# antgroup/ant-ray

Measured on NVIDIA H100. Metric: resnet50_ddp_train_images_per_sec, higher is better.
Workload: dtype bf16

## Files before the change

### ant-ray_b200/csrc/inst_norm.cu

```cuda
#include <algorithm>
#include <initializer_list>
#include <type_traits>

#include "norm_act.cuh"
#include "norm_cat.cuh"
#include "norm_infer.cuh"
#include "norm_kernels.cuh"
#include "norm_launch.h"
#include "norm_pool2.cuh"
#include "norm_res.cuh"
#include "norm_shuffle.cuh"
#include "norm_slice.cuh"

namespace b200c {
namespace bn {

static int ceil_div(int a, int b) { return (a + b - 1) / b; }

static int last_pow2(unsigned n) {
  n |= (n >> 1);
  n |= (n >> 2);
  n |= (n >> 4);
  n |= (n >> 8);
  n |= (n >> 16);
  return std::max<int>(1, n - (n >> 1));
}

static void reduce_config(int reduction, int stride, dim3* block, dim3* grid) {
  int block_x = std::min(last_pow2(stride), kTileW);
  int block_y = std::min(last_pow2(ceil_div(reduction, kElemsPerThread)), kMaxBlock / block_x);
  if (block_x * block_y != kMaxBlock) block_x = std::min(last_pow2(stride), kMaxBlock / block_y);
  int grid_y = std::min(ceil_div(reduction, block_y * kElemsPerThread), kMaxHBlock);
  *block = dim3(block_x, block_y, 1);
  *grid = dim3(ceil_div(stride, block_x), grid_y < 8 ? 1 : grid_y, 1);
}

static_assert(kEwVec % kStatsVec == 0, "vec_ok covers the statistics kernel's vector width");
static bool vec_ok(int stride, const void* const* ptrs, int n) {
  if (stride % kEwVec) return false;
  for (int i = 0; i < n; i++)
    if (reinterpret_cast<uintptr_t>(ptrs[i]) % 16) return false;
  return true;
}

constexpr size_t kBlockSmem = 48 * 1024;
constexpr size_t kStatsStaticSmem = 3 * kMaxBlock * 4 + 16;
constexpr size_t kBwdStaticSmem = 2 * kMaxBlock * 4 + 16;

static size_t stats_ring_bytes(dim3 block) {
  return (size_t)kStatsStages * kParallelLoads * block.x * block.y * sizeof(BVec<kStatsVec>);
}
static_assert(kStatsStaticSmem + (size_t)kStatsStages * kParallelLoads * (kMaxBlock / kStatsVec) * sizeof(BVec<kStatsVec>) <= kBlockSmem,
              "the statistics ring fits every block");

static_assert(kBwdStaticSmem + (size_t)kBwdStagesWide * 5 * kParallelLoads * (kMaxBlock / kBwdVec) * sizeof(BVec<kBwdVec>) <= kBlockSmem &&
                  kBwdStaticSmem + (size_t)kBwdStages * 2 * kParallelLoads * (kMaxBlock / kBwdVec) * sizeof(BVec<kBwdVec>) <= kBlockSmem,
              "the backward ring fits every block: 2 stages of up to 5 operands, 3 of 2");
struct BwdReduceLaunch {
  dim3 block, grid;
  int vec;
  size_t smem;
};
static BwdReduceLaunch bwd_reduce_launch(int m, int c, GradSrc src, bool dy2, bool dual, const void* const* ptrs, int n) {
  BwdReduceLaunch l;
  reduce_config(m, c, &l.block, &l.grid);
  l.vec = 1;
  l.smem = 0;
  if (src == kGradPool || !vec_ok(c, ptrs, n)) return l;
  const int ops = bwd_ring_operands(src == kGradY, dy2, dual);
  const size_t ring = (size_t)bwd_ring_stages(ops) * ops * kParallelLoads * (l.block.x / kBwdVec) * l.block.y * sizeof(BVec<kBwdVec>);
  l.block.x /= kBwdVec;
  l.vec = kBwdVec;
  l.smem = ring;
  return l;
}

static void ew_config(int reduction, int stride, int vec, dim3* block, dim3* grid) {
  const int groups = stride / vec;
  const int bx = std::min(groups, kEwThreads);
  const int by = kEwThreads / bx;
  const int gx = ceil_div(groups, bx);
  const int gy = std::max(1, std::min(ceil_div(reduction, by), 4096 / gx));
  *block = dim3(bx, by, 1);
  *grid = dim3(gx, gy, 1);
}

constexpr int kSemaphores = kMaxChannels / kTileW;
constexpr size_t kSemaphoreBytes = (size_t)kSemaphores * 4;

size_t scratch_bytes(int stride) {
  return kSemaphoreBytes + (size_t)3 * stride * kMaxHBlock * 4 + (size_t)2 * stride * 4;
}

struct Scratch {
  int* semaphores;
  float* staging;
  float* sums;
};
static Scratch carve(void* scratch, int stride) {
  char* p = static_cast<char*>(scratch);
  Scratch s;
  s.semaphores = reinterpret_cast<int*>(p);
  s.staging = reinterpret_cast<float*>(p + kSemaphoreBytes);
  s.sums = s.staging + (size_t)3 * stride * kMaxHBlock;
  return s;
}

template <int... Cs, typename F>
static auto with_const(int key, F&& f) {
  std::common_type_t<decltype(f(std::integral_constant<int, Cs>{}))...> kernel = nullptr;
  ((key == Cs ? void(kernel = f(std::integral_constant<int, Cs>{})) : void()), ...);
  return kernel;
}

using StatsKernel = void (*)(const bf16*, StatsOut, volatile float*, int*, int, int);
using SyncStatsKernel = void (*)(const bf16*, float*, float, volatile float*, int*, int, int);
using StatsDualKernel = void (*)(const bf16*, const bf16*, StatsOut, StatsOut, volatile float*, volatile float*, int*, int, int);
using TransformKernel = void (*)(const bf16*, const bf16*, bf16*, uint8_t*, const float*, const float*, const float*, const float*,
                                 const float*, const float*, const float*, const float*, int, int);
using PoolFwdKernel = void (*)(const bf16*, bf16*, uint8_t*, const float*, const float*, const float*, const float*, PoolDims, int, int);
using BwdReduceKernel = void (*)(const bf16*, const bf16*, const bf16*, const bf16*, const uint8_t*, bf16*, const float*, const float*,
                                 float*, float*, float*, float*, volatile float*, int*, PoolDims, const bf16*, const float*, const float*,
                                 float*, float*, float*, int, int, int);
using BwdElemtKernel = void (*)(const bf16*, const bf16*, const bf16*, const uint8_t*, const bf16*, bf16*, const float*, const float*,
                                const float*, const float*, const float*, const float*, float, const bf16*, bf16*, const float*,
                                const float*, const float*, const float*, int, int);

static StatsKernel stats_kernel(int vec) {
  return with_const<1, kStatsVec>(vec, [](auto v) -> StatsKernel { return k_bn_stats<decltype(v)::value>; });
}
static StatsDualKernel stats_dual_kernel(int vec) {
  return with_const<1, kStatsVec>(vec, [](auto v) -> StatsDualKernel { return k_bn_stats_dual<decltype(v)::value>; });
}
static SyncStatsKernel sync_stats_kernel(int vec) {
  return with_const<1, kStatsVec>(vec, [](auto v) -> SyncStatsKernel { return k_bn_sync_stats<decltype(v)::value>; });
}
static TransformKernel transform_kernel(int vec, int tail) {
  return with_const<1, kEwVec>(vec, [&](auto v) {
    return with_const<kTailNone, kTailRelu, kTailAddRelu, kTailBnAddRelu>(
        tail, [](auto t) -> TransformKernel { return k_bn_transform<decltype(v)::value, (Tail) decltype(t)::value>; });
  });
}
static PoolFwdKernel pool_fwd_kernel(int vec) {
  return with_const<1, kEwVec>(vec, [](auto v) -> PoolFwdKernel { return k_bn_pool_fwd<decltype(v)::value>; });
}
static BwdReduceKernel bwd_reduce_kernel(int src, bool dual) {
  if (dual)
    return with_const<kGradY, kGradBits>(src, [](auto g) -> BwdReduceKernel { return k_bn_bwd_reduce<(GradSrc) decltype(g)::value, true>; });
  return with_const<kGradY, kGradBits, kGradDy, kGradPool>(
      src, [](auto g) -> BwdReduceKernel { return k_bn_bwd_reduce<(GradSrc) decltype(g)::value, false>; });
}
static BwdElemtKernel bwd_elemt_kernel(int vec, int src, bool fct_ptr, bool dual) {
  return with_const<1, kEwVec>(vec, [&](auto v) {
    if (dual)
// ... 159 lines not shown
      if (vec == 1) load(act_bwd_reduce_kernel(act));
      load(act_transform_kernel(vec, act));
      load(act_infer_kernel<float>(vec, act));
      load(act_infer_kernel<bf16>(vec, act));
    }
    for (bool b : {false, true}) {
      load(res_transform_kernel(vec, b));
      load(res_infer_kernel<float>(vec, b));
      load(res_infer_kernel<bf16>(vec, b));
    }
  }
  return e;
}

constexpr cudaError_t kNoKernel = cudaErrorInvalidDeviceFunction;

static cudaError_t launch_stats(const FwdArgs& a, float* sync_row, cudaStream_t st) {
  Scratch s = carve(a.scratch, a.c);
  dim3 block, grid;
  reduce_config(a.m, a.c, &block, &grid);
  const int vec = vec_ok(a.c, &a.x, 1) ? kStatsVec : 1;
  block.x /= vec;
  const size_t smem = vec == kStatsVec ? stats_ring_bytes(block) : 0;
  const bf16* x = static_cast<const bf16*>(a.x);
  if (sync_row) {
    const SyncStatsKernel k = sync_stats_kernel(vec);
    if (!k) return kNoKernel;
    k<<<grid, block, smem, st>>>(x, sync_row, a.eps, s.staging, s.semaphores, a.m, a.c);
  } else {
    const StatsKernel k = stats_kernel(vec);
    if (!k) return kNoKernel;
    StatsOut o{a.save_mean, a.save_invstd, a.running_mean, a.running_var, a.num_batches_tracked, a.momentum,
               (float)((double)a.m / (double)(a.m - 1)), a.eps};
    k<<<grid, block, smem, st>>>(x, o, s.staging, s.semaphores, a.m, a.c);
  }
  return cudaGetLastError();
}

static cudaError_t launch_transform(const FwdArgs& a, cudaStream_t st) {
  const void* ptrs[3] = {a.x, a.y, a.identity ? a.identity : a.x};
  const int vec = vec_ok(a.c, ptrs, 3) ? kEwVec : 1;
  dim3 block, grid;
  ew_config(a.m, a.c, vec, &block, &grid);
  const TransformKernel k = transform_kernel(vec, !a.relu ? kTailNone : a.identity ? kTailAddRelu : kTailRelu);
  if (!k) return kNoKernel;
  k<<<grid, block, 0, st>>>(static_cast<const bf16*>(a.x), static_cast<const bf16*>(a.identity), static_cast<bf16*>(a.y),
                            static_cast<uint8_t*>(a.mask), a.save_mean, a.save_invstd, a.weight, a.bias, nullptr, nullptr, nullptr,
                            nullptr, a.m, a.c);
  return cudaGetLastError();
}

static PoolDims pool_dims(int h, int w) { return PoolDims{h, w, (h - 1) / 2 + 1, (w - 1) / 2 + 1}; }

static cudaError_t launch_pool_fwd(const FwdArgs& a, cudaStream_t st) {
  const PoolDims d = pool_dims(a.pool_h, a.pool_w);
  const int pooled_rows = a.m / (a.pool_h * a.pool_w) * d.oh * d.ow;
  const void* ptrs[3] = {a.x, a.y, a.argmax};
  const int vec = vec_ok(a.c, ptrs, 3) ? kEwVec : 1;
  dim3 block, grid;
  ew_config(pooled_rows, a.c, vec, &block, &grid);
  const PoolFwdKernel k = pool_fwd_kernel(vec);
  if (!k) return kNoKernel;
  k<<<grid, block, 0, st>>>(static_cast<const bf16*>(a.x), static_cast<bf16*>(a.y), static_cast<uint8_t*>(a.argmax), a.save_mean,
                            a.save_invstd, a.weight, a.bias, d, pooled_rows, a.c);
  return cudaGetLastError();
}

cudaError_t forward(const FwdArgs& a, cudaStream_t st) {
  const cudaError_t e = launch_stats(a, nullptr, st);
  if (e != cudaSuccess) return e;
  return a.pool_h ? launch_pool_fwd(a, st) : launch_transform(a, st);
}

static GradSrc grad_src(const BwdArgs& a, bool reduced) {
  if (!a.relu) return kGradDy;
  if (reduced && a.dy_masked) return kGradMasked;
  if (a.pool_h) return kGradPool;
  return a.mask ? kGradBits : kGradY;
}

static cudaError_t launch_bwd_reduce(const BwdArgs& a, cudaStream_t st) {
  Scratch s = carve(a.scratch, a.c);
  const GradSrc src = grad_src(a, false);
  const void* ptrs[5] = {a.x, a.dy, a.dy2 ? a.dy2 : a.dy, src == kGradY ? a.y : a.dy, a.dy_masked ? a.dy_masked : a.dy};
  const BwdReduceLaunch l = bwd_reduce_launch(a.m, a.c, src, a.dy2 != nullptr, false, ptrs, 5);
  const BwdReduceKernel k = bwd_reduce_kernel(src, false);
  if (!k) return kNoKernel;
  const void* mask = src == kGradPool ? a.argmax : a.mask;
  k<<<l.grid, l.block, l.smem, st>>>(static_cast<const bf16*>(a.x), static_cast<const bf16*>(a.dy), static_cast<const bf16*>(a.dy2),
                            static_cast<const bf16*>(a.y), static_cast<const uint8_t*>(mask), static_cast<bf16*>(a.dy_masked),
                            a.save_mean, a.save_invstd, s.sums, s.sums + a.c, a.grad_weight, a.grad_bias, s.staging, s.semaphores,
                            pool_dims(a.pool_h, a.pool_w), nullptr, nullptr, nullptr, nullptr, nullptr, nullptr, a.m, a.c, l.vec);
  return cudaGetLastError();
}

static cudaError_t launch_bwd_elemt(const BwdArgs& a, cudaStream_t st) {
  Scratch s = carve(a.scratch, a.c);
  const GradSrc src = grad_src(a, true);
  const void* g = src == kGradMasked ? a.dy_masked : a.dy;
  const void* ptrs[5] = {a.x, a.dx, g, a.dy2 && src != kGradMasked ? a.dy2 : a.dy, a.y};
  const int vec = vec_ok(a.c, ptrs, src == kGradY ? 5 : 4) ? kEwVec : 1;
  dim3 block, grid;
  ew_config(a.m, a.c, vec, &block, &grid);
  const BwdElemtKernel k = bwd_elemt_kernel(vec, src, a.norm_fct != nullptr, false);
  if (!k) return kNoKernel;
  k<<<grid, block, 0, st>>>(static_cast<const bf16*>(g), static_cast<const bf16*>(a.dy2), static_cast<const bf16*>(a.y),
                            static_cast<const uint8_t*>(a.mask), static_cast<const bf16*>(a.x), static_cast<bf16*>(a.dx), a.save_mean,
                            a.save_invstd, a.weight, s.sums, s.sums + a.c, a.norm_fct, (float)(1.0 / a.m), nullptr, nullptr, nullptr,
                            nullptr, nullptr, nullptr, a.m, a.c);
  return cudaGetLastError();
}

cudaError_t backward(const BwdArgs& a, cudaStream_t st) {
  const cudaError_t e = launch_bwd_reduce(a, st);
  return e == cudaSuccess ? launch_bwd_elemt(a, st) : e;
}

static size_t dual_extra_offset(int c) { return (scratch_bytes(c) + 15) / 16 * 16; }
size_t dual_scratch_bytes(int c) { return dual_extra_offset(c) + (size_t)3 * c * kMaxHBlock * 4 + (size_t)c * 4; }
static float* dual_staging(void* scratch, int c) { return reinterpret_cast<float*>(static_cast<char*>(scratch) + dual_extra_offset(c)); }
static float* dual_sum_xmu2(void* scratch, int c) { return dual_staging(scratch, c) + (size_t)3 * c * kMaxHBlock; }

static cudaError_t launch_stats_dual(const FwdArgs& a, const FwdArgs& b, cudaStream_t st) {
  Scratch s = carve(a.scratch, a.c);
  dim3 block, grid;
  reduce_config(a.m, a.c, &block, &grid);
  const void* xs[2] = {a.x, b.x};
  const int svec = vec_ok(a.c, xs, 2) ? kStatsVec : 1;
  block.x /= svec;
  grid.z = 2;
  const size_t smem = svec == kStatsVec ? stats_ring_bytes(block) : 0;
  const StatsDualKernel ks = stats_dual_kernel(svec);
  if (!ks) return kNoKernel;
  StatsOut oa{a.save_mean, a.save_invstd, a.running_mean, a.running_var, a.num_batches_tracked, a.momentum,
              (float)((double)a.m / (double)(a.m - 1)), a.eps};
  StatsOut ob{b.save_mean, b.save_invstd, b.running_mean, b.running_var, b.num_batches_tracked, b.momentum,
              (float)((double)b.m / (double)(b.m - 1)), b.eps};
  ks<<<grid, block, smem, st>>>(static_cast<const bf16*>(a.x), static_cast<const bf16*>(b.x), oa, ob, s.staging,
                             dual_staging(a.scratch, a.c), s.semaphores, a.m, a.c);
  return cudaGetLastError();
}

cudaError_t forward_dual(const FwdArgs& a, const FwdArgs& b, cudaStream_t st) {
  const cudaError_t e = launch_stats_dual(a, b, st);
  if (e != cudaSuccess) return e;
  dim3 block, grid;
  const void* ptrs[3] = {a.x, a.y, b.x};
  const int vec = vec_ok(a.c, ptrs, 3) ? kEwVec : 1;
  ew_config(a.m, a.c, vec, &block, &grid);
  const TransformKernel kt = transform_kernel(vec, kTailBnAddRelu);
  if (!kt) return kNoKernel;
  kt<<<grid, block, 0, st>>>(static_cast<const bf16*>(a.x), static_cast<const bf16*>(b.x), static_cast<bf16*>(a.y),
                             static_cast<uint8_t*>(a.mask), a.save_mean, a.save_invstd, a.weight, a.bias, b.save_mean, b.save_invstd,
                             b.weight, b.bias, a.m, a.c);
  return cudaGetLastError();
}

cudaError_t backward_dual(const BwdArgs& a, const BwdArgs& b, cudaStream_t st) {
  Scratch s = carve(a.scratch, a.c);
  float* sum2 = dual_sum_xmu2(a.scratch, a.c);
  const GradSrc src = a.mask ? kGradBits : kGradY;
  const void* rptrs[5] = {a.x, a.dy, a.dy2 ? a.dy2 : a.dy, src == kGradY ? a.y : a.dy, b.x};
  const BwdReduceLaunch l = bwd_reduce_launch(a.m, a.c, src, a.dy2 != nullptr, true, rptrs, 5);
  const BwdReduceKernel kr = bwd_reduce_kernel(src, true);
  if (!kr) return kNoKernel;
  kr<<<l.grid, l.block, l.smem, st>>>(static_cast<const bf16*>(a.x), static_cast<const bf16*>(a.dy), static_cast<const bf16*>(a.dy2),
                             static_cast<const bf16*>(a.y), static_cast<const uint8_t*>(a.mask), nullptr, a.save_mean, a.save_invstd,
                             s.sums, s.sums + a.c, a.grad_weight, a.grad_bias, s.staging, s.semaphores, pool_dims(0, 0),
// ... 439 lines not shown
```

### ant-ray_b200/csrc/norm_kernels.cuh

```cuda
#pragma once
#include <cuda_bf16.h>
#include <cuda_runtime.h>
#include <stdint.h>

#include <type_traits>

namespace b200c {
namespace bn {

constexpr int kMaxBlock = 512;
constexpr int kParallelLoads = 4;
constexpr int kElemsPerThread = 16;
constexpr int kTileW = 32;
constexpr int kMaxHBlock = 128;
constexpr int kStatsVec = 4;
constexpr int kBwdVec = 4;
constexpr int kStatsStages = 4;
constexpr unsigned kBwdStages = 3;
constexpr unsigned kBwdStagesWide = 2;
__host__ __device__ constexpr unsigned bwd_ring_stages(int ops) { return ops >= 3 ? kBwdStagesWide : kBwdStages; }
__host__ __device__ constexpr int bwd_ring_operands(bool y, bool dy2, bool dual) { return 2 + dy2 + y + dual; }
constexpr int kEwThreads = 256;
constexpr int kEwVec = 8;

typedef __nv_bfloat16 bf16;

template <int V>
struct alignas(2 * V) BVec {
  bf16 v[V];
};

__device__ __forceinline__ unsigned char* ring_smem() {
  extern __shared__ __align__(16) unsigned char bn_ring[];
  return bn_ring;
}
template <int BYTES>
__device__ __forceinline__ void cp_async(void* smem, const void* gmem) {
  asm volatile("cp.async.ca.shared.global [%0], [%1], %2;\n" ::"r"((unsigned)__cvta_generic_to_shared(smem)), "l"(gmem), "n"(BYTES)
               : "memory");
}
__device__ __forceinline__ void cp_async_commit() { asm volatile("cp.async.commit_group;\n" ::: "memory"); }
template <int N>
__device__ __forceinline__ void cp_async_wait() { asm volatile("cp.async.wait_group %0;\n" ::"n"(N) : "memory"); }


template <bool FUSE_NEW>
__device__ __forceinline__ void welford_merge_element(int& count, float& mean, float& m2n, const int& count_new,
                                                      const float& mean_new, const float& m2n_new) {
  float factor = float(1.0) / ::max(1, (count + count_new));
  float delta0 = mean - mean_new;
  const float c = count, c_new = count_new;
  mean = __fmul_rn(FUSE_NEW ? __fmaf_rn(mean_new, c_new, __fmul_rn(mean, c)) : __fmaf_rn(mean, c, __fmul_rn(mean_new, c_new)),
                   factor);
  m2n = __fadd_rn(m2n, __fmaf_rn(__fmul_rn(__fmul_rn(__fmul_rn(delta0, delta0), c_new), c), factor, m2n_new));
  count += count_new;
}

template <int V>
__device__ __forceinline__ void welford_merge_block_vertical(int (&count)[V], float (&mean)[V], float (&m2n)[V],
                                                             int* shmem_count, float* shmem_mean, float* shmem_m2n) {
  const int block_x = blockDim.x * V;
  auto address_base = threadIdx.x * V + threadIdx.y * block_x;
#pragma unroll
  for (int offset = blockDim.y / 2; offset > 0; offset >>= 1) {
    if (threadIdx.y < offset * 2) {
#pragma unroll
      for (int k = 0; k < V; k++) {
        shmem_mean[address_base + k] = mean[k];
        shmem_m2n[address_base + k] = m2n[k];
        shmem_count[address_base + k] = count[k];
      }
    }
    __syncthreads();
    if (threadIdx.y < offset && threadIdx.y + offset < blockDim.y) {
      auto address = address_base + offset * block_x;
#pragma unroll
      for (int k = 0; k < V; k++) {
        auto count_new = shmem_count[address + k];
        auto mean_new = shmem_mean[address + k];
        auto m2n_new = shmem_m2n[address + k];
        welford_merge_element<false>(count[k], mean[k], m2n[k], count_new, mean_new, m2n_new);
      }
    }
  }
}

template <int V>
__device__ __forceinline__ void merge_block_vertical_backward(float (&sum_dy)[V], float (&sum_dy_xmu)[V], float* shmem_sum_dy,
                                                              float* shmem_sum_dy_xmu) {
  const int block_x = blockDim.x * V;
  auto address_base = threadIdx.x * V + threadIdx.y * block_x;
#pragma unroll
  for (int offset = blockDim.y / 2; offset > 0; offset >>= 1) {
    if (threadIdx.y < offset * 2) {
#pragma unroll
      for (int k = 0; k < V; k++) {
        shmem_sum_dy[address_base + k] = sum_dy[k];
        shmem_sum_dy_xmu[address_base + k] = sum_dy_xmu[k];
      }
    }
    __syncthreads();
    if (threadIdx.y < offset && threadIdx.y + offset < blockDim.y) {
      auto address = address_base + offset * block_x;
// ... 304 lines not shown
#pragma unroll
    for (int j = 0; j < V; j++) {
      auto tmp = w_c[j] * (__bfloat162float(xv.v[j]) - m_c[j]) * inv_std_c[j] + s_c[j];
      if (TAIL == kTailAddRelu || BN2) {
        if (BN2) zv.v[j] = __float2bfloat16(w2_c[j] * (__bfloat162float(zv.v[j]) - m2_c[j]) * inv_std2_c[j] + s2_c[j]);
        const bf16 r = __float2bfloat16(__bfloat162float(__float2bfloat16(tmp)) + __bfloat162float(zv.v[j]));
        yv.v[j] = __bfloat162float(r) <= 0.f ? __float2bfloat16(0.f) : r;
      } else if (TAIL == kTailRelu) {
        yv.v[j] = tmp <= 0.f ? __float2bfloat16(0.f) : __float2bfloat16(tmp);
      } else {
        yv.v[j] = __float2bfloat16(tmp);
      }
      bits |= (unsigned)!(__bfloat162float(yv.v[j]) <= 0.f) << j;
    }
    *reinterpret_cast<BVec<V>*>(out + a) = yv;
    if (TAIL != kTailNone && mask) {
      if (V == 1) bits = (__ballot_sync(group, bits) >> (lane & ~7u)) & 0xffu;
      if (V == 8 || lane % 8 == 0) mask[a >> 3] = (uint8_t)bits;
    }
  }
}

struct PoolDims {
  int h, w, oh, ow;
};
constexpr uint8_t kPoolNoGrad = 0xff;

template <int V>
__global__ void __launch_bounds__(kEwThreads) k_bn_pool_fwd(const bf16* __restrict__ input, bf16* __restrict__ out,
                                                            uint8_t* __restrict__ argmax, const float* __restrict__ mean,
                                                            const float* __restrict__ inv_std, const float* __restrict__ weight,
                                                            const float* __restrict__ shift, const PoolDims d, const int pooled_rows,
                                                            const int stride) {
  const int c0 = (blockIdx.x * blockDim.x + threadIdx.x) * V;
  if (c0 >= stride) return;
  float m_c[V], inv_std_c[V], w_c[V], s_c[V];
#pragma unroll
  for (int j = 0; j < V; j++) {
    m_c[j] = mean[c0 + j];
    inv_std_c[j] = inv_std[c0 + j];
    w_c[j] = weight[c0 + j];
    s_c[j] = shift[c0 + j];
  }
  const int row_step = blockDim.y * gridDim.y;
  for (int p = blockIdx.y * blockDim.y + threadIdx.y; p < pooled_rows; p += row_step) {
    const int pw = p % d.ow, ph = (p / d.ow) % d.oh, n = p / (d.ow * d.oh);
    float best[V];
    uint8_t pos[V];
#pragma unroll
    for (int j = 0; j < V; j++) {
      best[j] = -INFINITY;
      pos[j] = 0;
    }
    for (int ih = max(2 * ph - 1, 0); ih < min(2 * ph + 2, d.h); ih++) {
      for (int iw = max(2 * pw - 1, 0); iw < min(2 * pw + 2, d.w); iw++) {
        const BVec<V> xv = *reinterpret_cast<const BVec<V>*>(input + ((size_t)(n * d.h + ih) * d.w + iw) * stride + c0);
        const uint8_t at = (ih - 2 * ph + 1) * 3 + (iw - 2 * pw + 1);
#pragma unroll
        for (int j = 0; j < V; j++) {
          const auto tmp = w_c[j] * (__bfloat162float(xv.v[j]) - m_c[j]) * inv_std_c[j] + s_c[j];
          const float y = __bfloat162float(tmp <= 0.f ? __float2bfloat16(0.f) : __float2bfloat16(tmp));
          if (y > best[j] || isnan(y)) {
            best[j] = y;
            pos[j] = at;
          }
        }
      }
    }
    BVec<V> yv;
    struct alignas(V) {
      uint8_t v[V];
    } av;
#pragma unroll
    for (int j = 0; j < V; j++) {
      yv.v[j] = __float2bfloat16(best[j]);
      av.v[j] = best[j] <= 0.f ? kPoolNoGrad : pos[j];
    }
    const size_t a = (size_t)p * stride + c0;
    *reinterpret_cast<BVec<V>*>(out + a) = yv;
    *reinterpret_cast<decltype(av)*>(argmax + a) = av;
  }
}

__device__ __forceinline__ bf16 pool_grad(const bf16* __restrict__ dpool, const uint8_t* __restrict__ argmax, const PoolDims& d,
                                          const int m, const int c, const int stride) {
  const int iw = m % d.w, ih = (m / d.w) % d.h, n = m / (d.w * d.h);
  const int ph0 = ih >> 1, ph1 = min((ih + 1) >> 1, d.oh - 1);
  const int pw0 = iw >> 1, pw1 = min((iw + 1) >> 1, d.ow - 1);
  const int o = ((n * d.oh + ph0) * d.ow + pw0) * stride + c;
  const int dr = (ph1 - ph0) * d.ow * stride, dc = (pw1 - pw0) * stride;
  const uint8_t a[4] = {argmax[o], argmax[o + dc], argmax[o + dr], argmax[o + dr + dc]};
  const bf16 v[4] = {dpool[o], dpool[o + dc], dpool[o + dr], dpool[o + dr + dc]};
  const int at = (ih - 2 * ph0 + 1) * 3 + (iw - 2 * pw0 + 1);
  if (ph0 == ph1 && pw0 == pw1) return a[0] == at ? v[0] : __float2bfloat16(0.f);
  float sum = 0.f;
  if (a[0] == at) sum += __bfloat162float(v[0]);
  if (pw1 != pw0 && a[1] == at - 2) sum += __bfloat162float(v[1]);
  if (ph1 != ph0 && a[2] == at - 6) sum += __bfloat162float(v[2]);
  if (ph1 != ph0 && pw1 != pw0 && a[3] == at - 8) sum += __bfloat162float(v[3]);
  return __float2bfloat16(sum);
}

__device__ __forceinline__ bf16 relu_grad(bf16 dy, bf16 y) { return __bfloat162float(y) <= 0.f ? __float2bfloat16(0.f) : dy; }
__device__ __forceinline__ bf16 relu_grad_bit(bf16 dy, unsigned bit) { return bit ? dy : __float2bfloat16(0.f); }
__device__ __forceinline__ bf16 add_grads(bf16 a, bf16 b) { return __float2bfloat16(__bfloat162float(a) + __bfloat162float(b)); }

enum GradSrc { kGradMasked, kGradY, kGradBits, kGradDy, kGradPool };
constexpr int kGradSrcs = 5;

template <GradSrc G, bool DUAL>
__global__ void __launch_bounds__(kMaxBlock) k_bn_bwd_reduce(const bf16* __restrict__ input, const bf16* __restrict__ grad_output,
                                const bf16* __restrict__ grad_output2, const bf16* __restrict__ output,
                                const uint8_t* __restrict__ mask, bf16* __restrict__ masked, const float* __restrict__ mean,
                                const float* __restrict__ inv_std, float* __restrict__ sum_dy_o, float* __restrict__ sum_dy_xmu_o,
                                float* __restrict__ grad_weight, float* __restrict__ grad_bias, volatile float* staging_data,
                                int* semaphores, const PoolDims pool, const bf16* __restrict__ input2,
                                const float* __restrict__ mean2, const float* __restrict__ inv_std2, float* __restrict__ sum_dy_xmu2_o,
                                float* __restrict__ grad_weight2, float* __restrict__ grad_bias2, const int reduction_size,
                                const int stride, const int vec) {
  static_assert(G != kGradMasked, "the reduce kernel computes g");
  constexpr bool BITS = G == kGradBits;
  constexpr bool POOL = G == kGradPool;
  constexpr int PARALLEL_LOADS = kParallelLoads;
  __shared__ float shmem_sum_dy[kMaxBlock];
  __shared__ float shmem_sum_dy_xmu[kMaxBlock];
  __shared__ bool is_last_block_done;

  auto body = [&](auto vec_c) {
    constexpr int V = decltype(vec_c)::value;
    float sum_dy[PARALLEL_LOADS][V];
    float sum_dy_xmu[PARALLEL_LOADS][V];
    float sum_dy_xmu2[PARALLEL_LOADS][V];
#pragma unroll
    for (int i = 0; i < PARALLEL_LOADS; i++) {
#pragma unroll
      for (int k = 0; k < V; k++) {
        sum_dy[i][k] = float(0);
        sum_dy_xmu[i][k] = float(0);
        sum_dy_xmu2[i][k] = float(0);
      }
    }
    int inner_loop_stride = blockDim.y * gridDim.y;
    int m_offset = blockIdx.y * blockDim.y + threadIdx.y;
    int c_offset = (blockIdx.x * blockDim.x + threadIdx.x) * V;
    if (c_offset >= stride || m_offset >= reduction_size) return;

    int loop_count = 1 + (reduction_size - 1) / (inner_loop_stride * PARALLEL_LOADS);
    int address_base = m_offset * stride + c_offset;
    int address_increment = inner_loop_stride * stride;
    float r_mean[V], factor[V], r_mean2[V];
#pragma unroll
    for (int k = 0; k < V; k++) {
      r_mean[k] = mean[c_offset + k];
      factor[k] = inv_std[c_offset + k];
      r_mean2[k] = DUAL ? mean2[c_offset + k] : 0.f;
    }

    auto consume = [&](int j, const BVec<V>* dy_p, const BVec<V>* dy2_p, const BVec<V>* y_p, uint8_t mask_byte, const BVec<V>* x_p,
                       const BVec<V>* x2_p) {
      float x_input[V], x_input2[V], x_grad_output[V];
      if (m_offset < reduction_size) {
        const unsigned bits = BITS ? mask_byte >> (address_base & 7) : 0u;
        BVec<V> gv;
#pragma unroll
        for (int k = 0; k < V; k++) {
          const bf16 dy = !POOL && grad_output2 ? add_grads(dy_p->v[k], dy2_p->v[k]) : dy_p->v[k];
          gv.v[k] = BITS ? relu_grad_bit(dy, (bits >> k) & 1u) : G == kGradY ? relu_grad(dy, y_p->v[k]) : dy;
          x_input[k] = __bfloat162float(x_p->v[k]);
          x_input2[k] = DUAL ? __bfloat162float(x2_p->v[k]) : 0.f;
          x_grad_output[k] = __bfloat162float(gv.v[k]);
        }
        if (masked) *reinterpret_cast<BVec<V>*>(masked + address_base) = gv;
      } else {
#pragma unroll
        for (int k = 0; k < V; k++) {
          x_input[k] = float(0);
          x_input2[k] = float(0);
          x_grad_output[k] = float(0);
        }
      }
      m_offset += inner_loop_stride;
      address_base += address_increment;
#pragma unroll
      for (int k = 0; k < V; k++) {
        sum_dy[j][k] += x_grad_output[k];
        sum_dy_xmu[j][k] = __fmaf_rn(x_grad_output[k], x_input[k] - r_mean[k], sum_dy_xmu[j][k]);
        if (DUAL) sum_dy_xmu2[j][k] = __fmaf_rn(x_grad_output[k], x_input2[k] - r_mean2[k], sum_dy_xmu2[j][k]);
      }
    };

    if constexpr (V == 1) {
      for (int i = 0; i < loop_count; i++) {
        BVec<V> dy_v[PARALLEL_LOADS], dy2_v[PARALLEL_LOADS], y_v[PARALLEL_LOADS], x_v[PARALLEL_LOADS], x2_v[PARALLEL_LOADS];
        uint8_t mask_v[PARALLEL_LOADS];
#pragma unroll
        for (int j = 0; j < PARALLEL_LOADS; j++) {
          if (m_offset + j * inner_loop_stride < reduction_size) {
            const int a = address_base + j * address_increment;
            if (POOL) dy_v[j].v[0] = pool_grad(grad_output, mask, pool, m_offset + j * inner_loop_stride, c_offset, stride);
            else dy_v[j].v[0] = grad_output[a];
            if (grad_output2) dy2_v[j].v[0] = grad_output2[a];
            if (BITS) mask_v[j] = mask[a >> 3];
            else if (G == kGradY) y_v[j].v[0] = output[a];
            x_v[j].v[0] = input[a];
            if (DUAL) x2_v[j].v[0] = input2[a];
          }
        }
#pragma unroll
        for (int j = 0; j < PARALLEL_LOADS; j++) consume(j, &dy_v[j], &dy2_v[j], &y_v[j], mask_v[j], &x_v[j], &x2_v[j]);
      }
    } else {
      const int ops = bwd_ring_operands(G == kGradY, grad_output2 != nullptr, DUAL);
      auto ring_walk = [&](auto stages_c) {
        constexpr unsigned D = decltype(stages_c)::value;
        const int threads = blockDim.x * blockDim.y;
        const int op_dy2 = 2, op_y = op_dy2 + (grad_output2 != nullptr), op_x2 = op_y + (G == kGradY);
        BVec<V>* ring = reinterpret_cast<BVec<V>*>(ring_smem()) + threadIdx.y * blockDim.x + threadIdx.x;
        auto stage = [&](unsigned it) { return ring + (it % D) * ops * PARALLEL_LOADS * threads; };
        const int first_row = m_offset;
        const int iteration_rows = PARALLEL_LOADS * inner_loop_stride;
        auto issue = [&](unsigned it) {
          BVec<V>* slot = stage(it);
          int m = first_row + (int)it * iteration_rows;
#pragma unroll
          for (int j = 0; j < PARALLEL_LOADS; j++, m += inner_loop_stride, slot += threads) {
            if (m < reduction_size) {
              const size_t a = (size_t)m * stride + c_offset;
              cp_async<sizeof(BVec<V>)>(slot, grad_output + a);
              cp_async<sizeof(BVec<V>)>(slot + PARALLEL_LOADS * threads, input + a);
              if (grad_output2) cp_async<sizeof(BVec<V>)>(slot + op_dy2 * PARALLEL_LOADS * threads, grad_output2 + a);
              if (G == kGradY) cp_async<sizeof(BVec<V>)>(slot + op_y * PARALLEL_LOADS * threads, output + a);
              if (DUAL) cp_async<sizeof(BVec<V>)>(slot + op_x2 * PARALLEL_LOADS * threads, input2 + a);
            }
          }
          cp_async_commit();
        };
        uint8_t mask_next[PARALLEL_LOADS];
        auto load_mask = [&](unsigned it) {
          int m = first_row + (int)it * iteration_rows;
#pragma unroll
          for (int j = 0; j < PARALLEL_LOADS; j++, m += inner_loop_stride)
            if (m < reduction_size) mask_next[j] = mask[((size_t)m * stride + c_offset) >> 3];
        };
        if (BITS) load_mask(0);
#pragma unroll
        for (unsigned it = 0; it < D - 1; it++) issue(it);
        for (unsigned i = 0; i < (unsigned)loop_count; i++) {
          issue(i + D - 1);
          uint8_t mask_v[PARALLEL_LOADS];
#pragma unroll
          for (int j = 0; j < PARALLEL_LOADS; j++) mask_v[j] = mask_next[j];
          if (BITS) load_mask(i + 1);
          cp_async_wait<D - 1>();
          const BVec<V>* slot = stage(i);
#pragma unroll
          for (int j = 0; j < PARALLEL_LOADS; j++, slot += threads)
            consume(j, slot, slot + op_dy2 * PARALLEL_LOADS * threads, slot + op_y * PARALLEL_LOADS * threads, mask_v[j],
                    slot + PARALLEL_LOADS * threads, slot + op_x2 * PARALLEL_LOADS * threads);
        }
      };
      if (DUAL || bwd_ring_stages(ops) == kBwdStagesWide) ring_walk(std::integral_constant<unsigned, kBwdStagesWide>{});
      else ring_walk(std::integral_constant<unsigned, kBwdStages>{});
    }

    float sum_dy_th[V], sum_dy_xmu_th[V], sum_dy_xmu2_th[V];
#pragma unroll
    for (int k = 0; k < V; k++) {
#pragma unroll
      for (int j = 1; j < PARALLEL_LOADS; j++) {
        sum_dy[0][k] += sum_dy[j][k];
        sum_dy_xmu[0][k] += sum_dy_xmu[j][k];
        if (DUAL) sum_dy_xmu2[0][k] += sum_dy_xmu2[j][k];
      }
      sum_dy_th[k] = sum_dy[0][k];
      sum_dy_xmu_th[k] = sum_dy_xmu[0][k];
      sum_dy_xmu2_th[k] = sum_dy_xmu2[0][k];
    }

    auto merge = [&]() {
      merge_block_vertical_backward<V>(sum_dy_th, sum_dy_xmu_th, shmem_sum_dy, shmem_sum_dy_xmu);
      if (DUAL) {
        __syncthreads();
        float unused[V] = {};
        merge_block_vertical_backward<V>(sum_dy_xmu2_th, unused, shmem_sum_dy, shmem_sum_dy_xmu);
      }
    };
    merge();

    auto write_sums = [&]() {
#pragma unroll
      for (int k = 0; k < V; k++) {
        const int c = c_offset + k;
        grad_bias[c] = sum_dy_th[k];
        grad_weight[c] = sum_dy_xmu_th[k] * factor[k];
        sum_dy_o[c] = sum_dy_th[k];
        sum_dy_xmu_o[c] = sum_dy_xmu_th[k];
        if (DUAL) {
          grad_bias2[c] = sum_dy_th[k];
          grad_weight2[c] = sum_dy_xmu2_th[k] * inv_std2[c];
          sum_dy_xmu2_o[c] = sum_dy_xmu2_th[k];
        }
      }
    };
    if (gridDim.y > 1) {
      volatile float* staging_sum_dy = staging_data;
      volatile float* staging_sum_dy_xmu = &staging_data[stride * gridDim.y];
      volatile float* staging_sum_dy_xmu2 = &staging_data[2 * stride * gridDim.y];
      address_base = c_offset + blockIdx.y * stride;
      if (threadIdx.y == 0 && c_offset < stride) {
#pragma unroll
        for (int k = 0; k < V; k++) {
          staging_sum_dy[address_base + k] = sum_dy_th[k];
          staging_sum_dy_xmu[address_base + k] = sum_dy_xmu_th[k];
          if (DUAL) staging_sum_dy_xmu2[address_base + k] = sum_dy_xmu2_th[k];
        }
      }
      __threadfence();
      __syncthreads();
      if (threadIdx.x == 0 && threadIdx.y == 0) {
        int old = atomicAdd(&semaphores[blockIdx.x], 1);
        is_last_block_done = (old == (gridDim.y - 1));
        if (is_last_block_done) semaphores[blockIdx.x] = 0;
      }
      __syncthreads();
      if (is_last_block_done) {
#pragma unroll
        for (int k = 0; k < V; k++) {
          sum_dy_th[k] = float(0.0);
          sum_dy_xmu_th[k] = float(0.0);
          sum_dy_xmu2_th[k] = float(0.0);
        }
        for (int y = threadIdx.y; y < gridDim.y; y += blockDim.y) {
          address_base = c_offset + y * stride;
#pragma unroll
          for (int k = 0; k < V; k++) {
            sum_dy_th[k] += (c_offset < stride ? staging_sum_dy[address_base + k] : float(0.0));
            sum_dy_xmu_th[k] += (c_offset < stride ? staging_sum_dy_xmu[address_base + k] : float(0.0));
            if (DUAL) sum_dy_xmu2_th[k] += (c_offset < stride ? staging_sum_dy_xmu2[address_base + k] : float(0.0));
          }
        }
        merge();
        if (threadIdx.y == 0 && c_offset < stride) write_sums();
      }
    } else {
      if (blockIdx.y == 0 && threadIdx.y == 0 && c_offset < stride) write_sums();
    }
  };
  if constexpr (POOL) body(std::integral_constant<int, 1>{});
  else if (vec == kBwdVec) body(std::integral_constant<int, kBwdVec>{});
  else body(std::integral_constant<int, 1>{});
}

template <int V, GradSrc G, bool FCT_PTR, bool DUAL>
__global__ void __launch_bounds__(kEwThreads) k_bn_bwd_elemt(const bf16* __restrict__ grad_output, const bf16* __restrict__ grad_output2,
                                                             const bf16* __restrict__ output, const uint8_t* __restrict__ mask,
                                                             const bf16* __restrict__ input, bf16* __restrict__ grad_input,
                                                             const float* __restrict__ mean, const float* __restrict__ inv_std,
                                                             const float* __restrict__ weight, const float* __restrict__ sum_dy,
                                                             const float* __restrict__ sum_dy_xmu,
                                                             const float* __restrict__ norm_fct_ptr, const float norm_fct_value,
                                                             const bf16* __restrict__ input2, bf16* __restrict__ grad_input2,
                                                             const float* __restrict__ mean2, const float* __restrict__ inv_std2,
                                                             const float* __restrict__ weight2, const float* __restrict__ sum_dy_xmu2,
                                                             const int reduction_size, const int stride) {
  static_assert(!DUAL || (G == kGradY || G == kGradBits), "a dual tail derives g from dy and the ReLU");
  const float norm_fct = FCT_PTR ? *norm_fct_ptr : norm_fct_value;
  const int c0 = (blockIdx.x * blockDim.x + threadIdx.x) * V;
  if (c0 >= stride) return;
  float m_c[V], m_dy_c[V], factor_1_c[V], factor_2_c[V];
  float m2_c[V], factor2_1_c[V], factor2_2_c[V];
#pragma unroll
  for (int j = 0; j < V; j++) {
    m_c[j] = mean[c0 + j];
    m_dy_c[j] = sum_dy[c0 + j] * norm_fct;
    factor_1_c[j] = inv_std[c0 + j];
    factor_2_c[j] = weight[c0 + j] * factor_1_c[j];
    factor_1_c[j] = factor_1_c[j] * factor_1_c[j] * sum_dy_xmu[c0 + j] * norm_fct;
    if (DUAL) {
      m2_c[j] = mean2[c0 + j];
      factor2_1_c[j] = inv_std2[c0 + j];
      factor2_2_c[j] = weight2[c0 + j] * factor2_1_c[j];
      factor2_1_c[j] = factor2_1_c[j] * factor2_1_c[j] * sum_dy_xmu2[c0 + j] * norm_fct;
    }
  }
  const int row_step = blockDim.y * gridDim.y;
  for (int m = blockIdx.y * blockDim.y + threadIdx.y; m < reduction_size; m += row_step) {
    const int a = m * stride + c0;
    const BVec<V> gv = *reinterpret_cast<const BVec<V>*>(grad_output + a);
    BVec<V> gv2, yv;
    if (G != kGradMasked && grad_output2) gv2 = *reinterpret_cast<const BVec<V>*>(grad_output2 + a);
    unsigned bits = 0;
    if (G == kGradY) yv = *reinterpret_cast<const BVec<V>*>(output + a);
    if (G == kGradBits) bits = mask[a >> 3] >> (a & 7);
    const BVec<V> xv = *reinterpret_cast<const BVec<V>*>(input + a);
    BVec<V> x2v, dxv, dx2v;
    if (DUAL) x2v = *reinterpret_cast<const BVec<V>*>(input2 + a);
#pragma unroll
    for (int j = 0; j < V; j++) {
      const bf16 dy = G != kGradMasked && grad_output2 ? add_grads(gv.v[j], gv2.v[j]) : gv.v[j];
      const float g = __bfloat162float(G == kGradMasked || G == kGradDy ? dy
                                       : G == kGradY ? relu_grad(dy, yv.v[j]) : relu_grad_bit(dy, (bits >> j) & 1u));
      dxv.v[j] = __float2bfloat16((g - m_dy_c[j] - (__bfloat162float(xv.v[j]) - m_c[j]) * factor_1_c[j]) * factor_2_c[j]);
      if (DUAL)
        dx2v.v[j] = __float2bfloat16((g - m_dy_c[j] - (__bfloat162float(x2v.v[j]) - m2_c[j]) * factor2_1_c[j]) * factor2_2_c[j]);
    }
    *reinterpret_cast<BVec<V>*>(grad_input + a) = dxv;
    if (DUAL) *reinterpret_cast<BVec<V>*>(grad_input2 + a) = dx2v;
  }
}

}
}
```

Baseline: 5640.

## Vectorize and cp.async-pipeline the stem BN backward reduce through max-pool gradient

The stem batch-norm backward reduce that reads its gradient through the max-pool argmax previously ran scalar (V=1) with no shared-memory ring. It now runs with 4-wide vectors and a 4-stage cp.async ring holding x, the primary pooled gradient and the argmax bytes. Neighbouring pool-window values are fetched into registers one iteration ahead, and row coordinates are advanced incrementally instead of recomputed with divisions. This targets memory latency and per-element index math in a bandwidth-bound kernel, at the cost of more registers, more shared memory and some extra irregular global loads.

```diff
diff --git a/ant-ray_b200/csrc/inst_norm.cu b/ant-ray_b200/csrc/inst_norm.cu
--- a/ant-ray_b200/csrc/inst_norm.cu
+++ b/ant-ray_b200/csrc/inst_norm.cu
@@ -56,6 +56,8 @@
 static_assert(kBwdStaticSmem + (size_t)kBwdStagesWide * 5 * kParallelLoads * (kMaxBlock / kBwdVec) * sizeof(BVec<kBwdVec>) <= kBlockSmem &&
                   kBwdStaticSmem + (size_t)kBwdStages * 2 * kParallelLoads * (kMaxBlock / kBwdVec) * sizeof(BVec<kBwdVec>) <= kBlockSmem,
               "the backward ring fits every block: 2 stages of up to 5 operands, 3 of 2");
+static_assert(kBwdStaticSmem + (size_t)kBwdPoolStages * kParallelLoads * (kMaxBlock / kBwdVec) * kBwdPoolRowBytes <= kBlockSmem,
+              "the stem's ring fits every block");
 struct BwdReduceLaunch {
   dim3 block, grid;
   int vec;
@@ -66,10 +68,12 @@
   reduce_config(m, c, &l.block, &l.grid);
   l.vec = 1;
   l.smem = 0;
-  if (src == kGradPool || !vec_ok(c, ptrs, n)) return l;
+  if (!vec_ok(c, ptrs, n)) return l;
+  l.block.x /= kBwdVec;
+  const size_t threads = (size_t)l.block.x * l.block.y;
   const int ops = bwd_ring_operands(src == kGradY, dy2, dual);
-  const size_t ring = (size_t)bwd_ring_stages(ops) * ops * kParallelLoads * (l.block.x / kBwdVec) * l.block.y * sizeof(BVec<kBwdVec>);
-  l.block.x /= kBwdVec;
+  const size_t ring = src == kGradPool ? kBwdPoolStages * kParallelLoads * threads * kBwdPoolRowBytes
+                                       : bwd_ring_stages(ops) * ops * kParallelLoads * threads * sizeof(BVec<kBwdVec>);
   l.vec = kBwdVec;
   l.smem = ring;
   return l;
@@ -395,8 +399,9 @@
 static cudaError_t launch_bwd_reduce(const BwdArgs& a, cudaStream_t st) {
   Scratch s = carve(a.scratch, a.c);
   const GradSrc src = grad_src(a, false);
-  const void* ptrs[5] = {a.x, a.dy, a.dy2 ? a.dy2 : a.dy, src == kGradY ? a.y : a.dy, a.dy_masked ? a.dy_masked : a.dy};
-  const BwdReduceLaunch l = bwd_reduce_launch(a.m, a.c, src, a.dy2 != nullptr, false, ptrs, 5);
+  const void* ptrs[6] = {a.x, a.dy, a.dy2 ? a.dy2 : a.dy, src == kGradY ? a.y : a.dy, a.dy_masked ? a.dy_masked : a.dy,
+                         src == kGradPool ? a.argmax : a.dy};
+  const BwdReduceLaunch l = bwd_reduce_launch(a.m, a.c, src, a.dy2 != nullptr, false, ptrs, 6);
   const BwdReduceKernel k = bwd_reduce_kernel(src, false);
   if (!k) return kNoKernel;
   const void* mask = src == kGradPool ? a.argmax : a.mask;
diff --git a/ant-ray_b200/csrc/norm_kernels.cuh b/ant-ray_b200/csrc/norm_kernels.cuh
--- a/ant-ray_b200/csrc/norm_kernels.cuh
+++ b/ant-ray_b200/csrc/norm_kernels.cuh
@@ -19,6 +19,8 @@
 constexpr unsigned kBwdStages = 3;
 constexpr unsigned kBwdStagesWide = 2;
 __host__ __device__ constexpr unsigned bwd_ring_stages(int ops) { return ops >= 3 ? kBwdStagesWide : kBwdStages; }
+constexpr unsigned kBwdPoolStages = 4;
+constexpr int kBwdPoolRowBytes = 2 * 2 * kBwdVec + kBwdVec;
 __host__ __device__ constexpr int bwd_ring_operands(bool y, bool dy2, bool dual) { return 2 + dy2 + y + dual; }
 constexpr int kEwThreads = 256;
 constexpr int kEwVec = 8;
@@ -489,6 +491,15 @@
   }
 }
 
+__device__ __forceinline__ bf16 pool_pick(const uint8_t (&a)[4], const bf16 (&v)[4], const int at, const bool row, const bool col) {
+  if (!row && !col) return a[0] == at ? v[0] : __float2bfloat16(0.f);
+  float sum = 0.f;
+  if (a[0] == at) sum += __bfloat162float(v[0]);
+  if (col && a[1] == at - 2) sum += __bfloat162float(v[1]);
+  if (row && a[2] == at - 6) sum += __bfloat162float(v[2]);
+  if (row && col && a[3] == at - 8) sum += __bfloat162float(v[3]);
+  return __float2bfloat16(sum);
+}
 __device__ __forceinline__ bf16 pool_grad(const bf16* __restrict__ dpool, const uint8_t* __restrict__ argmax, const PoolDims& d,
                                           const int m, const int c, const int stride) {
   const int iw = m % d.w, ih = (m / d.w) % d.h, n = m / (d.w * d.h);
@@ -499,13 +510,7 @@
   const uint8_t a[4] = {argmax[o], argmax[o + dc], argmax[o + dr], argmax[o + dr + dc]};
   const bf16 v[4] = {dpool[o], dpool[o + dc], dpool[o + dr], dpool[o + dr + dc]};
   const int at = (ih - 2 * ph0 + 1) * 3 + (iw - 2 * pw0 + 1);
-  if (ph0 == ph1 && pw0 == pw1) return a[0] == at ? v[0] : __float2bfloat16(0.f);
-  float sum = 0.f;
-  if (a[0] == at) sum += __bfloat162float(v[0]);
-  if (pw1 != pw0 && a[1] == at - 2) sum += __bfloat162float(v[1]);
-  if (ph1 != ph0 && a[2] == at - 6) sum += __bfloat162float(v[2]);
-  if (ph1 != ph0 && pw1 != pw0 && a[3] == at - 8) sum += __bfloat162float(v[3]);
-  return __float2bfloat16(sum);
+  return pool_pick(a, v, at, ph1 != ph0, pw1 != pw0);
 }
 
 __device__ __forceinline__ bf16 relu_grad(bf16 dy, bf16 y) { return __bfloat162float(y) <= 0.f ? __float2bfloat16(0.f) : dy; }
@@ -559,7 +564,7 @@
 #pragma unroll
     for (int k = 0; k < V; k++) {
       r_mean[k] = mean[c_offset + k];
-      factor[k] = inv_std[c_offset + k];
+      factor[k] = POOL && V > 1 ? 0.f : inv_std[c_offset + k];
       r_mean2[k] = DUAL ? mean2[c_offset + k] : 0.f;
     }
 
@@ -616,6 +621,110 @@
 #pragma unroll
         for (int j = 0; j < PARALLEL_LOADS; j++) consume(j, &dy_v[j], &dy2_v[j], &y_v[j], mask_v[j], &x_v[j], &x2_v[j]);
       }
+    } else if constexpr (POOL) {
+      constexpr unsigned D = kBwdPoolStages;
+      const int threads = blockDim.x * blockDim.y;
+      const int t = threadIdx.y * blockDim.x + threadIdx.x;
+      unsigned char* const ring = ring_smem();
+      const int stage_bytes = PARALLEL_LOADS * threads * kBwdPoolRowBytes;
+      auto x_slot = [&](unsigned it, int j) { return reinterpret_cast<BVec<V>*>(ring + (it % D) * stage_bytes) + j * threads + t; };
+      auto dp_slot = [&](unsigned it, int j) { return x_slot(it, j) + PARALLEL_LOADS * threads; };
+      auto am_slot = [&](unsigned it, int j) {
+        return reinterpret_cast<uint32_t*>(ring + (it % D) * stage_bytes + 2 * PARALLEL_LOADS * threads * sizeof(BVec<V>)) + j * threads + t;
+      };
+      struct Row {
+        int n, ih, iw;
+      };
+      const int dq = inner_loop_stride / pool.w, dw = inner_loop_stride - dq * pool.w;
+      const int dn = dq / pool.h, dh = dq - dn * pool.h;
+      auto step = [&](Row& r) {
+        r.iw += dw;
+        if (r.iw >= pool.w) {
+          r.iw -= pool.w;
+          r.ih++;
+        }
+        r.ih += dh;
+        if (r.ih >= pool.h) {
+          r.ih -= pool.h;
+          r.n++;
+        }
+        r.n += dn;
+      };
+      Row first;
+      const int q = m_offset / pool.w;
+      first.iw = m_offset - q * pool.w;
+      first.n = q / pool.h;
+      first.ih = q - first.n * pool.h;
+      auto row_index = [&](const Row& r) { return (r.n * pool.h + r.ih) * pool.w + r.iw; };
+      auto window0 = [&](const Row& r) { return ((r.n * pool.oh + (r.ih >> 1)) * pool.ow + (r.iw >> 1)) * stride + c_offset; };
+
+      Row issue_row = first;
+      auto issue = [&](unsigned it) {
+#pragma unroll
+        for (int j = 0; j < PARALLEL_LOADS; j++, step(issue_row)) {
+          const int m = row_index(issue_row);
+          if (m < reduction_size) {
+            const int o = window0(issue_row);
+            cp_async<sizeof(BVec<V>)>(x_slot(it, j), input + ((size_t)m * stride + c_offset));
+            cp_async<sizeof(BVec<V>)>(dp_slot(it, j), grad_output + o);
+            cp_async<4>(am_slot(it, j), mask + o);
+          }
+        }
+        cp_async_commit();
+      };
+      BVec<V> other_dp[PARALLEL_LOADS][3] = {};
+      uint32_t other_am[PARALLEL_LOADS][3] = {};
+      uint32_t shapes = 0;
+      Row other_row = first;
+      auto load_other = [&](int j) {
+        if (row_index(other_row) < reduction_size) {
+          const bool row = (other_row.ih & 1) && other_row.ih + 1 < pool.h, col = (other_row.iw & 1) && other_row.iw + 1 < pool.w;
+          const uint32_t shape = 4 + 3 * (other_row.ih & 1) + (other_row.iw & 1) + 16 * row + 32 * col;
+          shapes = (shapes & ~(0xffu << 8 * j)) | shape << 8 * j;
+          const int o = window0(other_row), dr = pool.ow * stride;
+          if (col) {
+            other_dp[j][0] = *reinterpret_cast<const BVec<V>*>(grad_output + o + stride);
+            other_am[j][0] = *reinterpret_cast<const uint32_t*>(mask + o + stride);
+          }
+          if (row) {
+            other_dp[j][1] = *reinterpret_cast<const BVec<V>*>(grad_output + o + dr);
+            other_am[j][1] = *reinterpret_cast<const uint32_t*>(mask + o + dr);
+          }
+          if (row && col) {
+            other_dp[j][2] = *reinterpret_cast<const BVec<V>*>(grad_output + o + dr + stride);
+            other_am[j][2] = *reinterpret_cast<const uint32_t*>(mask + o + dr + stride);
+          }
+        }
+        step(other_row);
+      };
+#pragma unroll
+      for (unsigned it = 0; it < D - 1; it++) issue(it);
+#pragma unroll
+      for (int j = 0; j < PARALLEL_LOADS; j++) load_other(j);
+      for (unsigned i = 0; i < (unsigned)loop_count; i++) {
+        issue(i + D - 1);
+        cp_async_wait<D - 1>();
+#pragma unroll
+        for (int j = 0; j < PARALLEL_LOADS; j++) {
+          const BVec<V> dp0 = *dp_slot(i, j);
+          const uint32_t am0 = *am_slot(i, j);
+          const uint32_t shape = shapes >> 8 * j;
+          const int at = shape & 15;
+          const bool row = shape & 16, col = shape & 32;
+          BVec<V> gv;
+#pragma unroll
+          for (int k = 0; k < V; k++) {
+            const uint8_t a[4] = {(uint8_t)(am0 >> 8 * k), (uint8_t)(other_am[j][0] >> 8 * k), (uint8_t)(other_am[j][1] >> 8 * k),
+                                  (uint8_t)(other_am[j][2] >> 8 * k)};
+            const bf16 v[4] = {dp0.v[k], other_dp[j][0].v[k], other_dp[j][1].v[k], other_dp[j][2].v[k]};
+            gv.v[k] = pool_pick(a, v, at, row, col);
+          }
+          consume(j, &gv, nullptr, nullptr, 0, x_slot(i, j), nullptr);
+          load_other(j);
+        }
+      }
+#pragma unroll
+      for (int k = 0; k < V; k++) factor[k] = inv_std[c_offset + k];
     } else {
       const int ops = bwd_ring_operands(G == kGradY, grad_output2 != nullptr, DUAL);
       auto ring_walk = [&](auto stages_c) {
@@ -753,8 +862,7 @@
       if (blockIdx.y == 0 && threadIdx.y == 0 && c_offset < stride) write_sums();
     }
   };
-  if constexpr (POOL) body(std::integral_constant<int, 1>{});
-  else if (vec == kBwdVec) body(std::integral_constant<int, kBwdVec>{});
+  if (vec == kBwdVec) body(std::integral_constant<int, kBwdVec>{});
   else body(std::integral_constant<int, 1>{});
 }
 
```

Result: no change. 5639, median of 6 (-0.0%).
